# AlibabaResearch/recom

Measured on AMD Instinct MI355X. Metric: inference QPS + p50 latency, 1000-col synth model, batch 512, 1×MI355X, higher is better.
Workload: dtype f32; 1 GPU; S2: 1000 cols, dims 8/16/32/64, vocab 1000000, B 512, 1 id/row, 10% bucketize-f32, ids uniform; batch=512, columns=1000, table_bytes=120000000000, serve_workers=1, arena_ring=1

## Files before the change

### recom_amd/csrc/fcp_bench_main.hip

```cpp
#include <hip/hip_runtime.h>

#include <algorithm>
#include <atomic>
#include <thread>
#include <chrono>
#include <cmath>
#include <cstdint>
#include <cstdio>
#include <cstdlib>
#include <cstring>
#include <string>
#include <vector>

#include "../../include/fcp_hip.h"
#include "numa_util.h"

struct fcp_harness;
extern "C" int fcp_harness_create(fcp_plan_t *, const fcp_process_args_t *, int, int, int, fcp_harness **);
extern "C" int fcp_harness_run(fcp_harness *, int, double *, float *, float *);
extern "C" int fcp_harness_destroy(fcp_harness *);
extern "C" int fcp_harness_copy_probe(size_t, int, float *);
extern "C" int fcp_harness_bw_probe(int, size_t, int, float *);
extern "C" int fcp_harness_gather_probe(size_t, int, int, int, float *, double *);

#define CHECK_HIP(e)                                                                        \
  do {                                                                                      \
    hipError_t e_ = (e);                                                                    \
    if (e_ != hipSuccess) {                                                                 \
      std::fprintf(stderr, "%s:%d %s: %s\n", __FILE__, __LINE__, #e, hipGetErrorString(e_)); \
      std::exit(1);                                                                         \
    }                                                                                       \
  } while (0)
#define CHECK_FCP(e)                                                                                \
  do {                                                                                              \
    int s_ = (e);                                                                                   \
    if (s_) {                                                                                       \
      std::fprintf(stderr, "%s:%d %s: %s (%s)\n", __FILE__, __LINE__, #e, fcp_status_string(s_),   \
                   fcp_last_error());                                                               \
      std::exit(1);                                                                                 \
    }                                                                                               \
  } while (0)

__host__ __device__ inline float hash_elem(uint32_t seed, uint64_t r, uint32_t e) {
  uint64_t u = (r * 2654435761ull + (uint64_t)e * 40503ull + ((seed * 7919u + 12345u) & 0xFFFFFFFFull)) & 0xFFFFFFFFull;
  u ^= u >> 15;
  u = (u * 0x2C1B3C6Dull) & 0xFFFFFFFFull;
  u ^= u >> 12;
  u = (u * 0x297A2D39ull) & 0xFFFFFFFFull;
  u ^= u >> 15;
  return (float)(u >> 8) * 1.1920928955078125e-07f - 1.0f;
}

struct BigArg { char bytes[640]; };
__global__ void noop_big_kernel(BigArg a) { if (a.bytes[0] == 77) __builtin_trap(); }
__global__ void noop_kernel(int *p) { if (p) *p = 1; }

__global__ void fill_table(float *t, uint32_t seed, uint64_t vocab, uint32_t dim) {
  const uint64_t n = vocab * dim;
  for (uint64_t i = (uint64_t)blockIdx.x * blockDim.x + threadIdx.x; i < n; i += (uint64_t)gridDim.x * blockDim.x)
    t[i] = hash_elem(seed, i / dim, (uint32_t)(i % dim));
}

static uint64_t splitmix(uint64_t &s) {
  uint64_t z = (s += 0x9E3779B97F4A7C15ull);
  z = (z ^ (z >> 30)) * 0xBF58476D1CE4E5B9ull;
  z = (z ^ (z >> 27)) * 0x94D049BB133111EBull;
  return z ^ (z >> 31);
}

static int bucketize_host(const std::vector<float> &b, float v) {
  int l = 0, r = (int)b.size() - 1;
  while (l <= r) {
    int mid = (l + r) >> 1;
    if (v < b[mid]) r = mid - 1; else l = mid + 1;
  }
  return r + 1;
}

static void *plain_alloc(void *ctx, size_t bytes) {
  void **slot = static_cast<void **>(ctx);
  if (hipMalloc(slot, bytes) != hipSuccess) return nullptr;
  return *slot;
}

int main(int argc, char **argv) {
  int columns = 1000, batch = 512, steps = 300, warmup = 50, threads = 1, requests = 16, ring = 6, verify = 1;
  int bucketize_every = 10;
  int slab = 0;
  int h2d = 0;
  int narrow = 0;
  int zero_copy = std::getenv("FCP_STAGER_ZERO_COPY") ? 1 : 0;
  int fixed_dim = 0;
  int pack_threads = 8;
  int stager_depth = 4;
  int copy_kernel = 1;
  long vocab = 1000000;
  for (int i = 1; i + 1 < argc; i += 2) {
    std::string k = argv[i];
    long v = std::atol(argv[i + 1]);
    if (k == "--columns") columns = (int)v;
    else if (k == "--batch") batch = (int)v;
    else if (k == "--vocab") vocab = v;
    else if (k == "--steps") steps = (int)v;
    else if (k == "--warmup") warmup = (int)v;
    else if (k == "--threads") threads = (int)v;
    else if (k == "--requests") requests = (int)v;
    else if (k == "--ring") ring = (int)v;
    else if (k == "--verify") verify = (int)v;
    else if (k == "--bucketize-every") bucketize_every = (int)v;
    else if (k == "--slab") slab = (int)v;
    else if (k == "--h2d") h2d = (int)v;
    else if (k == "--narrow") narrow = (int)v;
    else if (k == "--zero-copy") zero_copy = (int)v;
    else if (k == "--dim") fixed_dim = (int)v;
    else if (k == "--pack-threads") pack_threads = (int)v;
    else if (k == "--stager-depth") stager_depth = (int)v;
    else if (k == "--copy-kernel") copy_kernel = (int)v;
    else if (k == "--bw-probe") {
      const char *names[4] = {"read", "write", "write-nt", "chunked-write-nt"};
      for (int kind = 0; kind < 4; ++kind) {
        float ms = 0;
        const size_t bytes = (size_t)v << 20;
        fcp_harness_bw_probe(kind, bytes, 20, &ms);
        std::printf("%s probe %ld MiB: %.1f GB/s  (%.2f us)\n", names[kind], v, bytes / (ms * 1e-3) / 1e9, ms * 1e3);
      }
      return 0;
    }
    else if (k == "--gather-probe") {
      for (int row_bytes : {32, 64, 128, 256}) {
        for (int depth : {4, 8}) {
          float ms = 0;
          double useful = 0;
          fcp_harness_gather_probe((size_t)v << 20, row_bytes, depth, 10, &ms, &useful);
          std::printf("gather probe %ld MiB, %3d-byte rows, %d in flight: %.1f GB/s useful (%.2f us per launch)\n", v, row_bytes,
                      depth, useful / (ms * 1e-3) / 1e9, ms * 1e3);
        }
      }
      return 0;
    }
    else if (k == "--api-probe") {
      hipStream_t s1, s2;
      hipEvent_t e1, e2;
      CHECK_HIP(hipStreamCreateWithFlags(&s1, hipStreamNonBlocking));
      CHECK_HIP(hipStreamCreateWithFlags(&s2, hipStreamNonBlocking));
      CHECK_HIP(hipEventCreateWithFlags(&e1, hipEventDisableTiming));
      CHECK_HIP(hipEventCreateWithFlags(&e2, hipEventDisableTiming));
      const int n = (int)v;
      auto now = [] { return std::chrono::steady_clock::now(); };
      auto us = [&](std::chrono::steady_clock::time_point a) { return std::chrono::duration<double, std::micro>(now() - a).count() / n; };
      {
        hipFunction_t f = nullptr;
        CHECK_HIP(hipGetFuncBySymbol(&f, reinterpret_cast<const void *>(noop_big_kernel)));
        BigArg arg;
        std::memset(&arg, 0, sizeof(arg));
        size_t arg_size = sizeof(arg);
        void *extra[] = {HIP_LAUNCH_PARAM_BUFFER_POINTER, &arg, HIP_LAUNCH_PARAM_BUFFER_SIZE, &arg_size, HIP_LAUNCH_PARAM_END};
        auto t = now();
        for (int i = 0; i < n; ++i) hipLaunchKernelGGL(noop_big_kernel, dim3(1), dim3(64), 0, s1, arg);
        std::printf("hipLaunchKernelGGL, 640-byte argument    %.2f us\n", us(t));
        CHECK_HIP(hipStreamSynchronize(s1));
        t = now();
        for (int i = 0; i < n; ++i) CHECK_HIP(hipModuleLaunchKernel(f, 1, 1, 1, 64, 1, 1, 0, s1, nullptr, extra));
        std::printf("hipModuleLaunchKernel, same argument     %.2f us\n", us(t));
        CHECK_HIP(hipStreamSynchronize(s1));
      }
      auto t = now();
      for (int i = 0; i < n; ++i) hipLaunchKernelGGL(noop_kernel, dim3(1), dim3(64), 0, s1, nullptr);
      std::printf("kernel launch          %.2f us\n", us(t));
      CHECK_HIP(hipDeviceSynchronize());
      t = now();
// ... 117 lines not shown
        } else {
          int64_t id = (int64_t)(splitmix(rng) % (uint64_t)vocab);
          std::memcpy(p + 8 * b, &id, 8);
        }
      }
    }
    CHECK_HIP(hipMalloc(&d_blobs[v], size));
    CHECK_HIP(hipMemcpy(d_blobs[v], blobs[v].data(), size, hipMemcpyHostToDevice));
    fcp_process_args_t &a = variants[v];
    std::memset(&a, 0, sizeof(a));
    a.concated_inputs = d_blobs[v];
    a.concated_bytes = (int64_t)size;
    a.concated_offsets = offs[v].data();
    a.concated_shapes = shps[v].data();
    a.input_ptrs = tables.data();
  }

  if (verify) {
    void *arena = nullptr;
    fcp_process_args_t a = variants[0];
    a.malloc_buff = plain_alloc;
    a.malloc_buff_ctx = &arena;
    std::vector<void *> gp(1);
    std::vector<int32_t> gs(2);
    fcp_process_result_t res;
    std::memset(&res, 0, sizeof(res));
    res.group_ptrs = gp.data();
    res.group_shapes = gs.data();
    CHECK_FCP(fcp_process_feature_columns(plan, &a, &res));
    CHECK_HIP(hipDeviceSynchronize());
    const size_t W = gs[1];
    std::vector<float> out((size_t)batch * W);
    CHECK_HIP(hipMemcpy(out.data(), gp[0], out.size() * 4, hipMemcpyDeviceToHost));
    size_t bad = 0, off = 0;
    for (int c = 0; c < columns; ++c) {
      const char *p = blobs[0].data() + offs[0][c];
      for (int b = 0; b < batch; ++b) {
        int64_t id;
        if (esz[c] == 4) {
          float x;
          std::memcpy(&x, p + 4 * b, 4);
          id = bucketize_host(boundaries, x);
        } else {
          std::memcpy(&id, p + 8 * b, 8);
        }
        for (int e = 0; e < cols[c].dim; ++e)
          if (out[(size_t)b * W + off + e] != hash_elem(1000 + c, (uint64_t)id, e)) ++bad;
      }
      off += cols[c].dim;
    }
    std::printf("verify: %zu mismatching elements of %zu\n", bad, out.size());
    CHECK_HIP(hipFree(arena));
    if (bad) return 3;
  }

  if (h2d) {
    {
      cpu_set_t near;
      if (!std::getenv("FCP_STAGER_NO_PIN") && fcp::cpus_near_device(0, &near)) (void)sched_setaffinity(0, sizeof(near), &near);
    }
    std::vector<uint8_t> nflags(columns, 0);
    size_t shipped = blobs[0].size();
    if (narrow) {
      shipped = 0;
      for (int c = 0; c < columns; ++c) {
        if (cols[c].id_source == FCP_IDS_I64) {
          cols[c].id_source = FCP_IDS_I32;
          esz[c] = 4;
          nflags[c] = 1;
        }
        shipped += (size_t)batch * 4;
      }
      CHECK_FCP(fcp_plan_destroy(plan));
      CHECK_FCP(fcp_plan_create(&pd, &plan));
      for (int c = 0; c < columns; ++c)
        if (nflags[c]) esz[c] = 8;
    }
    std::vector<std::vector<fcp_host_tensor_t>> host(requests, std::vector<fcp_host_tensor_t>(columns));
    std::vector<int64_t> dims(1, batch);
    for (int v = 0; v < requests; ++v)
      for (int c = 0; c < columns; ++c) host[v][c] = {blobs[v].data() + offs[v][c], esz[c], 1, dims.data()};
    int64_t arena_bytes = 0;
    CHECK_FCP(fcp_plan_arena_bytes(plan, shps[0].data(), nullptr, &arena_bytes));
    struct RingCtx { std::vector<void *> *r; size_t i; };
    struct Worker {
      fcp_stager_t *st = nullptr;
      hipStream_t stream = nullptr;
      std::vector<void *> ring;
      RingCtx rc{nullptr, 0};
      double host_stage_us = 0, host_process_us = 0;
    };
    const int nw = threads < 1 ? 1 : threads;
    std::vector<Worker> W(nw);
    for (Worker &w : W) {
      CHECK_FCP(fcp_stager_create_ex(0, (int64_t)blobs[0].size() + 4096, columns, columns, stager_depth, pack_threads,
                                     zero_copy ? FCP_STAGER_ZERO_COPY : copy_kernel ? FCP_STAGER_COPY_KERNEL : FCP_STAGER_COPY_SDMA, &w.st));
      w.ring.resize(6);
      for (auto &p : w.ring) CHECK_HIP(hipMalloc(&p, (size_t)arena_bytes));
      w.rc.r = &w.ring;
      CHECK_HIP(hipStreamCreateWithFlags(&w.stream, hipStreamNonBlocking));
    }
    auto one = [&](Worker &w, int k) {
      const int v = k % requests;
      fcp_process_args_t a;
      std::memset(&a, 0, sizeof(a));
      const auto h0 = std::chrono::steady_clock::now();
// ... 105 lines not shown
```

### recom_amd/csrc/fcp_dense_plain.hip

```cpp
#include "fcp_fused_bodies.h"

namespace {

template <int R> struct PlainLds {
  static constexpr int RB = FCP_WAVES_PER_BLOCK * R;
  static constexpr int IDS = RB + 1;
  static constexpr int REC = sizeof(FcpPlainSpan) + FCP_WAVE * sizeof(FcpPlainCol);
  alignas(16) char rec[REC];
  uint32_t off[FCP_WAVE * IDS];
};
static_assert(sizeof(FcpPlainCol) == 48 && sizeof(FcpPlainSpan) == 80, "span records: 80-byte head, 48-byte columns");

typedef uint32_t __attribute__((ext_vector_type(2))) U2;
typedef U2 __attribute__((aligned(4))) Id64;

template <int R>
__global__ void __launch_bounds__(FCP_BLOCK_THREADS)
fcp_dense_kernel_plain(const char *img, const char *blob, float *out, unsigned long long *bad_ids, int rows, int nslots,
                       int nsp8, int nlist, int img_stride, int out_stride, int policy) {
  constexpr int V = 4, RB = PlainLds<R>::RB, IDS = PlainLds<R>::IDS;
  __shared__ PlainLds<R> S;
  const int tid = threadIdx.x;
  const int lane = tid & (FCP_WAVE - 1);
  const int wave = tid >> 6;

  const int bid = blockIdx.x;
  int idx, tile;
  if (nsp8 > 0) {
    const int xcd = bid & 7, j8 = bid >> 3;
    idx = (j8 % nsp8) * 8 + xcd;
    tile = j8 / nsp8;
  } else {
    idx = bid % (-nsp8);
    tile = bid / (-nsp8);
  }
  if (idx >= nlist) return;
  const int q0 = idx * FCP_WAVE, row_blk = tile * RB;
  if (q0 >= nslots || row_blk >= rows) return;

  typedef uint32_t __attribute__((ext_vector_type(4))) U4;
  {
    const FCP_GLOBAL U4 *g = as_global(reinterpret_cast<const U4 *>(img + (int64_t)idx * img_stride));
    if (tid < (img_stride >> 4)) reinterpret_cast<U4 *>(S.rec)[tid] = g[tid];
  }
  __syncthreads();
  const FcpPlainSpan &H = *reinterpret_cast<const FcpPlainSpan *>(S.rec);
  const FcpPlainCol *cols = reinterpret_cast<const FcpPlainCol *>(S.rec + sizeof(FcpPlainSpan));

  const int npairs = H.ncols * RB;
  for (int p = tid; p < npairs; p += FCP_BLOCK_THREADS) {
    const int j = p / RB, r = p % RB;
    const int b = row_blk + r;
    uint32_t off = kNoRow;
    if (b < rows) {
      const FcpPlainCol &c = cols[j];
      const char *a = blob + c.ids_off;
      const uint32_t kind = c.kind;
      int64_t id;
      if (kind == FCP_IDS_I64) {
        const Id64 w = ((const FCP_GLOBAL Id64 *)a)[b];
        id = (int64_t)(((uint64_t)w.y << 32) | w.x);
      } else {
        const uint32_t w = *as_global(reinterpret_cast<const uint32_t *>(a) + b);
        id = kind == FCP_IDS_F32_BUCKETIZE ? (int64_t)bucketize_arith(c.n_boundaries, c.bnd_b0, c.bnd_inv, c.bnd_step, __uint_as_float(w))
                                           : (int64_t)(int32_t)w;
      }
      const bool bad = (uint64_t)id >= (uint64_t)c.vocab;
      off = bad ? kBadRow : (uint32_t)id * c.spr;
      if (bad && bad_ids && c.out_off >= q0 * V) atomicAdd(bad_ids, 1ull);
    }
    S.off[j * IDS + r] = off;
  }
  __syncthreads();
  const int q = q0 + lane;
  if (q >= nslots) return;

  const int j = H.lane_col[lane];
  const float *tb = cols[j].table + (q * V - cols[j].out_off);
  float *outp = out + q * V;
  const int r0 = wave * R;
  uint32_t off[R];
#pragma unroll
  for (int r = 0; r < R; ++r) off[r] = S.off[j * IDS + r0 + r];
  VF<V> v[R];
#pragma unroll
  for (int r = 0; r < R; ++r) {
    v[r] = vzero<V>();
    if (is_row(off[r])) v[r] = ld_slot32<V>(tb, off[r]);
  }
#pragma unroll
  for (int r = 0; r < R; ++r) {
    const int b = row_blk + r0 + r;
    if (b < rows) st_out<V>(outp + (int64_t)b * out_stride, v[r], policy);
  }
}

}

int fcp_launch_dense_plain(const FcpPlainLaunch &P, int grid_blocks, ihipStream_t *s) {
  if (grid_blocks <= 0) return 0;
  if (P.img_stride <= 0 || (P.img_stride & 15) || P.img_stride > PlainLds<4>::REC) return (int)hipErrorInvalidValue;
  void *stop = nullptr;
  int flags = 0;
  fcp_take_launch_extras(&stop, &flags);
  const dim3 grid(grid_blocks), block(FCP_BLOCK_THREADS);
  if (stop || flags)
    hipExtLaunchKernelGGL(fcp_dense_kernel_plain<4>, grid, block, 0, s, nullptr, static_cast<hipEvent_t>(stop), flags, P.img, P.blob,
                          P.out, P.bad_ids, P.rows, P.nslots, P.nsp8, P.nlist, P.img_stride, P.out_stride, P.store_policy);
  else
    hipLaunchKernelGGL(fcp_dense_kernel_plain<4>, grid, block, 0, s, P.img, P.blob, P.out, P.bad_ids, P.rows, P.nslots, P.nsp8,
                       P.nlist, P.img_stride, P.out_stride, P.store_policy);
  return (int)hipGetLastError();
}
```

### recom_amd/csrc/fcp_host.h

```cpp
#pragma once
#include <hip/hip_runtime.h>
#include <hip/hip_ext.h>

#include <algorithm>
#include <atomic>
#include <chrono>
#include <cmath>
#include <cstdio>
#include <cstdlib>
#include <cstring>
#include <functional>
#include <map>
#include <memory>
#include <mutex>
#include <new>
#include <string>
#include <thread>
#include <vector>

#include "../../include/fcp_hip.h"
#include "fcp_internal.h"
#include "fcp_env.h"

namespace fcph {
// ... 121 lines not shown
};
void sup_reset(LaneSupervisor &S, const fcp::Env &env);
LanePool *lane_pool_for(int device);

struct PendingResult {
  uintptr_t end;
  hipEvent_t done;
  const void *owner;
};
void pending_register(const void *owner, void *arena, int64_t bytes, const void *blob, int64_t blob_bytes, hipEvent_t done);
void pending_clear_range(void *arena, int64_t bytes);
void pending_forget(const void *owner);
int stager_input_wait(const void *base, int64_t bytes, hipStream_t stream);
int stager_input_synchronize(const void *base, int64_t bytes);
int wait_for_inputs(const void *const *inputs, int32_t n, void *stream);

}
using namespace fcph;

struct fcp_plan {
  fcp::Env env;
  fcp_plan_desc_t desc;
  std::vector<HostColumn> cols;
  std::vector<int32_t> ranks, elem_sizes, shape_off;
  std::vector<int32_t> group_width, group_nslots, group_map_off;
  std::vector<int32_t> seg_cols;
  int32_t n_seg_plain = 0;
  bool seg_search = false;
  bool has_inverse = false;
  bool csr_by_pos = false;
  std::vector<int32_t> order, pos_of;
  struct FastCol {
    int32_t ids_input, seg_input, rows_arg, dim, seg_stride;
    int64_t out_off_bytes;
    uint8_t form, rows_source, seg_kind, group;
  };
  std::vector<FastCol> fast_cols;
  std::vector<int32_t> group_rep;
  int vec = 1;
  bool dense_only = true;
  std::vector<uint32_t> span_list;
  std::vector<int32_t> list_off[2], list_n[2];
  uint32_t *d_span_list = nullptr;
  bool host_only = false;
  int32_t rank_sum = 0;

  uint32_t *d_slot_map = nullptr;
  FcpColStatic *d_cols = nullptr;
  FcpXform *d_xforms = nullptr;
  FcpSegMap *d_segmaps = nullptr;
  bool has_seg_map = false;
  bool has_weights = false, weighted_kernel = false;
  bool plain_dense = false;
  int32_t plain_stride = 0, plain_spans = 0;
  std::vector<char> plain_tmpl;
  std::vector<std::pair<uint32_t, int32_t>> plain_entries;
  std::atomic<int32_t> last_dense_front{0};
  bool wide_rows = false;
  int out_kind = FCP_OUT_F32, out_elem = 4;
  int tab_kind = FCP_TAB_F32, tab_elem = 4;
  int tab_row_tail = 0;
  std::vector<FcpColStatic> h_cols;
  char *d_const = nullptr;
  int32_t *d_seg_cols = nullptr;
  unsigned long long *d_bad = nullptr;
  float *d_zeros = nullptr;
  std::vector<const void *> bound_tables;
  bool tables_bound = false;

  bool host_writes_dyn = false;
  std::mutex mu;
  DynSlot slots[kSlots];
  uint64_t tick = 0;

  LanePool *pool = nullptr;
  uint32_t lane_flags = 0;
  std::vector<std::pair<void *, bool>> lane_verdicts;
  std::atomic<void *> lane_good_caller{nullptr};
  int32_t lane_count = 0;
  std::atomic<bool> lane_relies{false};
  std::atomic<int64_t> last_work_bytes{0};
  int64_t lane_min_work = 0;
  int32_t request_order = FCP_ORDER_STREAM;
  std::atomic<uintptr_t> recent_arena[2] = {};
  struct LastLaunch {
    std::atomic<int32_t> kernel{0}, rows_per_wave{0}, store_policy{0}, dense_blocks{0}, ragged_blocks{0}, segment_offsets{0};
    std::atomic<int64_t> csr_arena_off{-1};
    std::unique_ptr<std::atomic<int32_t>[]> csr_base;
  } last_launch;
  std::atomic<bool> lane_demoted{false};
  LaneSupervisor sup;
  std::atomic<bool> sup_window{false};
};

namespace fcph {

struct DeviceGuard {
  int prev = -1;
  bool changed = false;
  int enter(int dev) {
    hipError_t e = hipGetDevice(&prev);
    if (e != hipSuccess) return hip_fail("hipGetDevice", e);
    if (prev != dev) {
      e = hipSetDevice(dev);
      if (e != hipSuccess) return hip_fail("hipSetDevice", e);
      changed = true;
    }
// ... 45 lines not shown
```

### recom_amd/csrc/fcp_internal.h

```cpp
#pragma once
#include <stddef.h>
#include <stdint.h>

#ifndef FCP_MAX_GROUPS
#define FCP_MAX_GROUPS 16
#endif
#define FCP_BLOCK_THREADS 256
#define FCP_WAVES_PER_BLOCK 4
#define FCP_WAVE 64

#define FCP_F_FORM(f) ((f) & 0xFu)
#define FCP_F_COMBINER(f) (((f) >> 4) & 0xFu)
#define FCP_F_IDSRC(f) (((f) >> 8) & 0xFu)
#define FCP_F_SEGKIND(f) (((f) >> 12) & 0xFu)
#define FCP_F_PACK(form, comb, idsrc, segkind) \
  ((uint32_t)(form) | ((uint32_t)(comb) << 4) | ((uint32_t)(idsrc) << 8) | ((uint32_t)(segkind) << 12))

struct FcpColStatic {
  const float *table;
  const float *boundaries;
  int64_t vocab;
  int32_t dim;
  int32_t out_off;
  uint32_t flags;
// ... 23 lines not shown
  int32_t inner;
  int32_t rows;
  int32_t seg_sym;
};

struct FcpSegMap {
  int64_t mul[4];
  int64_t div;
  int32_t n;
  int32_t sym_slot;
};

struct FcpGroupLaunch {
  int32_t rows;
  int32_t nslots;
  int32_t nsp8;
  int32_t block_begin;
  int32_t slot_map_off;
  int32_t span_list_off;
  int32_t nlist;
  int32_t csr_reg_stride;
};

struct FcpLaunch {
  const uint32_t *slot_map;
  const uint32_t *span_list;
  const FcpColStatic *cols;
  const FcpColDyn *dyn;
  const char *blob;
  char *arena;
  unsigned long long *bad_ids;
  int64_t csr_arena_off;
  int32_t n_groups;
  int32_t rows_per_wave;
  int32_t shard_rank, shard_world;
  int32_t seg_search;
  int32_t store_through;
  const int32_t *csr_reg;
  FcpGroupLaunch groups[FCP_MAX_GROUPS];
  const FcpXform *xforms;
  const float *zeros;
};

struct FcpPlainCol {
  const float *table;
  int64_t ids_off;
  uint32_t vocab;
  uint32_t spr;
  int32_t out_off;
  uint32_t kind;
  int32_t n_boundaries;
  float bnd_b0, bnd_inv, bnd_step;
};
struct FcpPlainSpan {
  int32_t ncols;
  int32_t pad_[3];
  uint8_t lane_col[FCP_WAVE];
};
struct FcpPlainLaunch {
  const char *img;
  const char *blob;
  float *out;
  unsigned long long *bad_ids;
  int32_t rows, nslots, nsp8, nlist;
  int32_t img_stride;
  int32_t out_stride;
  int32_t store_policy;
};

struct FcpSegLaunch {
  const int32_t *seg_cols;
  const FcpColStatic *cols;
  const FcpColDyn *dyn;
  const char *blob;
  char *arena;
  int64_t csr_arena_off;
  unsigned long long *bad_ids;
  const FcpXform *xforms;
  const FcpSegMap *segmaps;
  int32_t skip_inverse;
};

struct ihipStream_t;
void fcp_set_stop_event(void *event);
bool fcp_stop_event_pending();
void fcp_set_any_order(bool on);
int fcp_launch_fused(const FcpLaunch &L, int vec, bool dense_kernel, int grid_blocks, ihipStream_t *s);
int fcp_launch_hybrid(const FcpLaunch &Ldense, int dense_blocks, const FcpLaunch &Lragged, int ragged_blocks, int vec,
                      ihipStream_t *s);
int fcp_launch_weighted(const FcpLaunch &L, const int64_t *wts, int vec, int grid_blocks, ihipStream_t *s);
int fcp_launch_narrow(const FcpLaunch &L, int vec, bool dense_kernel, int out_kind, int grid_blocks, ihipStream_t *s);
int fcp_launch_narrow_hybrid(const FcpLaunch &Ldense, int dense_blocks, const FcpLaunch &Lragged, int ragged_blocks, int vec,
                             int out_kind, ihipStream_t *s);
int fcp_launch_tab16(const FcpLaunch &L, int vec, bool dense_kernel, int tab_kind, int grid_blocks, ihipStream_t *s);
int fcp_launch_tab16_hybrid(const FcpLaunch &Ldense, int dense_blocks, const FcpLaunch &Lragged, int ragged_blocks, int vec,
                            int tab_kind, ihipStream_t *s);
int fcp_launch_tabq8(const FcpLaunch &L, int vec, bool dense_kernel, int grid_blocks, ihipStream_t *s);
int fcp_launch_tabq8_hybrid(const FcpLaunch &Ldense, int dense_blocks, const FcpLaunch &Lragged, int ragged_blocks, int vec,
                            ihipStream_t *s);
int fcp_launch_dense_plain(const FcpPlainLaunch &P, int grid_blocks, ihipStream_t *s);
void fcp_take_launch_extras(void **stop_event, int *flags);
int fcp_launch_upload(const void *host_mapped_src, void *dst, size_t bytes, ihipStream_t *s);
int fcp_launch_h2d_copy(const void *host_mapped_src, void *dst, size_t bytes, ihipStream_t *s);
int fcp_launch_segment_offsets(const FcpSegLaunch &L, int n_seg_cols, int max_nnz, ihipStream_t *s, bool any_order = false);
int fcp_launch_concat_outputs(const void *const *inputs, const int32_t *dims, const int32_t *col_offsets, const int32_t *in_strides,
                              int32_t n, int64_t prefix, int32_t width, int32_t first_off, void *out,
                              ihipStream_t *s);
int fcp_launch_shard_finalize(const FcpLaunch &L, int group, const float *partials, int world,
                              int64_t row_begin, int64_t row_count, float *out, int vec,
// ... 2 lines not shown
```

### recom_amd/csrc/fcp_plan.hip

```cpp
#include "fcp_host.h"

namespace fcph {

thread_local std::string g_last_error;

int hip_fail(const char *what, hipError_t e) {
  g_last_error = std::string(what) + ": " + hipGetErrorString(e);
  return (e == hipErrorNoDevice || e == hipErrorInvalidDevice || e == hipErrorNoBinaryForGpu ||
          e == hipErrorInsufficientDriver)
             ? FCP_ERR_NO_DEVICE
             : FCP_ERR_HIP;
}

int fail(int code, const std::string &msg) {
  g_last_error = msg;
  return code;
}

}

int fcp_internal_fail(int code, const std::string &msg) { return fail(code, msg); }

namespace fcph {

// ... 538 lines not shown
    return std::min(std::max(g, 0), n);
  };
  auto exact = [&](float x) { return (int)(std::upper_bound(b.begin(), b.end(), x) - b.begin()); };
  int misses = 0;
  for (int i = 0; i < n; ++i) {
    if (i && !(b[i] > b[i - 1])) return;
    const float below = std::nextafter(b[i], -INFINITY);
    misses += guess(b[i]) != exact(b[i]);
    misses += guess(below) != exact(below);
  }
  if (misses * 8 > n) return;
  *b0 = lo;
  *inv = scale;
  const float step = b[1] - b[0];
  if (!(step > 0.0f) || !std::isfinite(step)) return;
  for (int i = 0; i < n; ++i)
    if (std::fmaf((float)i, step, lo) != b[i]) return;
  *step_out = step;
}

void build_plain_template(fcp_plan *p) {
  p->plain_dense = false;
  if (fcp::diag_ll("dense_generic", 0) != 0) return;
  const fcp_plan_desc_t &d = p->desc;
  if (p->out_elem != 4 || p->tab_elem != 4 || d.layout != FCP_LAYOUT_CONCAT || d.n_groups != 1 || d.shard_world > 1 || p->vec != 4 || p->wide_rows ||
      p->weighted_kernel || !p->dense_only || p->cols.empty())
    return;
  const int nc = (int)p->cols.size();
  for (int pos = 0; pos < nc; ++pos) {
    const HostColumn &hc = p->cols[p->order[pos]];
    const FcpColStatic &s = p->h_cols[pos];
    if (hc.d.form != FCP_FORM_GATHER || s.xform != 0 || hc.d.vocab < 0 || hc.d.vocab >= 0xFFFFFFFDLL) return;
    if (hc.d.id_source == FCP_IDS_F32_BUCKETIZE) {
      if (s.bnd_step == 0.0f) return;
    } else if (hc.d.id_source != FCP_IDS_I32 && hc.d.id_source != FCP_IDS_I64) {
      return;
    }
  }
  const int nslots = p->group_nslots[0];
  const int nspans = (nslots + FCP_WAVE - 1) / FCP_WAVE;
  if (p->list_n[0][0] != nspans) return;
  std::vector<int> first(nspans, nc), last(nspans, -1);
  for (int pos = 0; pos < nc; ++pos) {
    const FcpColStatic &s = p->h_cols[pos];
    const int s0 = s.out_off / 4 / FCP_WAVE, s1 = (s.out_off + s.dim - 1) / 4 / FCP_WAVE;
    for (int sp = s0; sp <= s1; ++sp) {
      first[sp] = std::min(first[sp], pos);
      last[sp] = std::max(last[sp], pos);
    }
  }
  int max_cols = 1;
  for (int sp = 0; sp < nspans; ++sp) max_cols = std::max(max_cols, last[sp] - first[sp] + 1);
  if (max_cols > FCP_WAVE) return;
  p->plain_stride = (int32_t)(sizeof(FcpPlainSpan) + (size_t)max_cols * sizeof(FcpPlainCol));
  p->plain_spans = nspans;
  p->plain_tmpl.assign((size_t)nspans * p->plain_stride, 0);
  p->plain_entries.clear();
  for (int sp = 0; sp < nspans; ++sp) {
    char *rec = p->plain_tmpl.data() + (size_t)sp * p->plain_stride;
    FcpPlainSpan head;
    std::memset(&head, 0, sizeof(head));
    head.ncols = last[sp] - first[sp] + 1;
    for (int pos = first[sp]; pos <= last[sp]; ++pos) {
      const FcpColStatic &s = p->h_cols[pos];
      FcpPlainCol c;
      std::memset(&c, 0, sizeof(c));
      c.table = nullptr;
      c.ids_off = 0;
      c.vocab = (uint32_t)s.vocab;
      c.spr = (uint32_t)(s.dim / 4);
      c.out_off = s.out_off;
      c.kind = FCP_F_IDSRC(s.flags);
      c.n_boundaries = s.n_boundaries;
      c.bnd_b0 = s.bnd_b0;
      c.bnd_inv = s.bnd_inv;
      c.bnd_step = s.bnd_step;
      const size_t at = (size_t)sp * p->plain_stride + sizeof(FcpPlainSpan) + (size_t)(pos - first[sp]) * sizeof(FcpPlainCol);
      std::memcpy(p->plain_tmpl.data() + at, &c, sizeof(c));
      p->plain_entries.emplace_back((uint32_t)at, pos);
      for (int q = std::max(s.out_off / 4, sp * FCP_WAVE); q < std::min((s.out_off + s.dim) / 4, (sp + 1) * FCP_WAVE); ++q)
        head.lane_col[q - sp * FCP_WAVE] = (uint8_t)(pos - first[sp]);
    }
    std::memcpy(rec, &head, sizeof(head));
  }
  p->plain_dense = true;
}

void destroy_device(fcp_plan *p) {
  if (p->host_only) return;
  for (auto &s : p->slots) {
    if (s.h_dyn) (void)hipHostFree(s.h_dyn);
    if (s.d_dyn) (void)hipFree(s.d_dyn);
    if (s.uploaded) (void)hipEventDestroy(s.uploaded);
    for (auto &e : s.done_pool) (void)hipEventDestroy(e.second);
  }
  if (p->d_slot_map) (void)hipFree(p->d_slot_map);
  if (p->d_span_list) (void)hipFree(p->d_span_list);
  if (p->d_cols) (void)hipFree(p->d_cols);
  if (p->d_xforms) (void)hipFree(p->d_xforms);
  if (p->d_segmaps) (void)hipFree(p->d_segmaps);
  if (p->d_const) (void)hipFree(p->d_const);
  if (p->d_seg_cols) (void)hipFree(p->d_seg_cols);
  if (p->d_bad) (void)hipFree(p->d_bad);
  if (p->d_zeros) (void)hipFree(p->d_zeros);
}

int init_device(fcp_plan *p) {
  DeviceGuard guard;
  int rc = guard.enter(p->desc.device);
  if (rc) return rc;
  const int nc = (int)p->cols.size();
  std::vector<uint32_t> map;
  for (int g = 0; g < p->desc.n_groups; ++g) {
    p->group_map_off[g] = (int32_t)map.size();
    for (int pos = 0; pos < nc; ++pos) {
      const HostColumn &hc = p->cols[p->order[pos]];
      if (hc.d.concat_group != g) continue;
      for (int s = 0; s < hc.d.dim / p->vec; ++s) map.push_back((uint32_t)pos);
    }
  }
  HIP_TRY(hipMalloc(&p->d_span_list, std::max<size_t>(p->span_list.size(), 1) * sizeof(uint32_t)));
  HIP_TRY(hipMemcpy(p->d_span_list, p->span_list.data(), p->span_list.size() * sizeof(uint32_t), hipMemcpyHostToDevice));
  HIP_TRY(hipMalloc(&p->d_slot_map, std::max<size_t>(map.size(), 1) * sizeof(uint32_t)));
  HIP_TRY(hipMemcpy(p->d_slot_map, map.data(), map.size() * sizeof(uint32_t), hipMemcpyHostToDevice));
  int64_t const_bytes = 0;
  std::vector<int> owners;
  for (size_t k = 0; k < p->cols.size(); ++k) {
    HostColumn &hc = p->cols[k];
    if (hc.boundaries.empty()) continue;
    for (int o : owners)
// ... 806 lines not shown
```

### recom_amd/csrc/fcp_process.hip

```cpp
#include "fcp_host.h"

namespace fcph {

bool stream_is_capturing(hipStream_t stream) {
  hipStreamCaptureStatus st = hipStreamCaptureStatusNone;
  if (stream && hipStreamIsCapturing(stream, &st) == hipSuccess) return st == hipStreamCaptureStatusActive;
  (void)hipGetLastError();
  return false;
}

static void fill_plain_image(const fcp_plan *p, const FcpColStatic *cols, FcpColDyn *h_dyn) {
  char *img = reinterpret_cast<char *>(h_dyn) + slot_image_off(p);
  std::memcpy(img, p->plain_tmpl.data(), p->plain_tmpl.size());
  for (const auto &e : p->plain_entries) {
    FcpPlainCol *c = reinterpret_cast<FcpPlainCol *>(img + e.first);
    c->table = cols[e.second].table;
    c->ids_off = h_dyn[e.second].ids_off;
  }
}

int bind_tables(fcp_plan *p, const void *const *input_ptrs, bool capturing) {
  const int nt = p->desc.n_device_inputs;
  if (p->tables_bound && std::memcmp(p->bound_tables.data(), input_ptrs, nt * sizeof(void *)) == 0)
    return FCP_OK;
  if (capturing)
    return fail(FCP_ERR_UNSUPPORTED, "stream capture of a request whose tables are not bound to the plan yet (or have moved): run it "
                                     "once on this stream before capturing");
  std::vector<FcpColStatic> cols = p->h_cols;
  for (size_t k = 0; k < p->cols.size(); ++k) {
    const int t = p->cols[k].d.table_input;
    const bool lookup = p->cols[k].d.form == FCP_FORM_GATHER || p->cols[k].d.form == FCP_FORM_SEGMENT_REDUCE ||
                        p->cols[k].d.form == FCP_FORM_GATHER_SCATTER;
    if (lookup) {
      const bool empty_shard = p->desc.shard_world > 1 && p->cols[k].d.vocab <= p->desc.shard_rank;
      if (!input_ptrs[t] && !empty_shard) return fail(FCP_ERR_INVALID_ARGUMENT, "null table pointer");
      cols[p->pos_of[k]].table = static_cast<const float *>(input_ptrs[t]);
    }
  }
  if (p->tables_bound) HIP_TRY(hipDeviceSynchronize());
  p->tables_bound = false;
  HIP_TRY(hipMemcpy(p->d_cols, cols.data(), cols.size() * sizeof(FcpColStatic), hipMemcpyHostToDevice));
  p->h_cols.swap(cols);
  if (p->plain_dense) {
    for (auto &s : p->slots) {
      if (!s.img_built) continue;
      fill_plain_image(p, p->h_cols.data(), s.h_dyn);
      const size_t off = slot_image_off(p);
      HIP_TRY(hipMemcpy(reinterpret_cast<char *>(s.d_dyn) + off, reinterpret_cast<const char *>(s.h_dyn) + off, p->plain_tmpl.size(),
                        hipMemcpyHostToDevice));
    }
  }
  for (int t = 0; t < nt; ++t) p->bound_tables[t] = input_ptrs[t];
  p->tables_bound = true;
  return FCP_OK;
}

int done_event_for(DynSlot &s, void *stream) {
  s.done_gen = 0;
  for (auto &e : s.done_pool)
    if (e.first == stream) {
      s.done = e.second;
      return FCP_OK;
    }
  hipEvent_t ev = nullptr;
  HIP_TRY(hipEventCreateWithFlags(&ev, hipEventDisableTiming | hipEventDisableSystemFence));
  s.done_pool.emplace_back(stream, ev);
  s.done = ev;
  return FCP_OK;
}

void build_key(const fcp_plan *p, const fcp_process_args_t *a, std::vector<int32_t> &key) {
  const int nh = (int)p->ranks.size();
  const int nsym = a->symbols ? p->desc.n_symbols : 0;
  const size_t key_len = (size_t)nh + p->rank_sum + nsym + 3;
  key.resize(key_len);
  std::memcpy(key.data(), a->concated_offsets, nh * sizeof(int32_t));
  std::memcpy(key.data() + nh, a->concated_shapes, p->rank_sum * sizeof(int32_t));
  if (nsym) std::memcpy(key.data() + nh + p->rank_sum, a->symbols, nsym * sizeof(int32_t));
  key[key_len - 3] = (int32_t)std::min<int64_t>(a->concated_bytes, 0x7fffffff);
  const uint64_t stream_bits = (uint64_t)reinterpret_cast<uintptr_t>(a->stream);
  key[key_len - 2] = (int32_t)(uint32_t)stream_bits;
  key[key_len - 1] = (int32_t)(uint32_t)(stream_bits >> 32);
}

int find_or_reserve(fcp_plan *p, const std::vector<int32_t> &key, DynSlot **out, bool *install, bool capturing) {
  ++p->tick;
  DynSlot *victim = nullptr;
  int pinned = 0;
  for (auto &s : p->slots) {
    if (s.valid && s.key == key) {
      s.tick = p->tick;
      ++s.users;
      ++s.uses;
      s.done_valid = false;
      if (capturing) s.captured = true;
      *out = &s;
      *install = false;
      return FCP_OK;
    }
    if (s.captured) {
      ++pinned;
      continue;
    }
    if (s.users > 0) continue;
    auto rank = [](const DynSlot &x) { return !x.valid ? 0 : (x.done_valid ? 1 : 2); };
    if (!victim || rank(s) < rank(*victim) || (rank(s) == rank(*victim) && s.tick < victim->tick)) victim = &s;
  }
  if (capturing) return kNeedsInstall;
  if (!victim)
    return pinned == kSlots ? fail(FCP_ERR_UNSUPPORTED, "every descriptor slot belongs to a captured graph: fcp_plan_release_captures")
                            : kAllSlotsBusy;
  victim->was_valid = victim->valid;
  victim->img_built = false;
  victim->valid = false;
  victim->users = 1;
  *out = victim;
  *install = true;
  return FCP_OK;
}

int install_slot(fcp_plan *p, const fcp_process_args_t *a, DynSlot &s) {
  hipStream_t stream = static_cast<hipStream_t>(a->stream);
  if (s.was_valid) {
    if (!s.done_valid) {
      if (s.stream == a->stream) {
        HIP_TRY(hipStreamSynchronize(stream));
      } else {
        HIP_TRY(hipDeviceSynchronize());
      }
    } else if (s.done_gen != 0 && s.done_gen != g_lane_generation.load(std::memory_order_acquire)) {
    } else if (hipEventQuery(s.done) != hipSuccess) {
      HIP_TRY(hipEventSynchronize(s.done));
    }
    if (!p->host_writes_dyn && hipEventQuery(s.uploaded) != hipSuccess) HIP_TRY(hipEventSynchronize(s.uploaded));
  }
  int rc = compute_dyn(p, a->concated_offsets, a->concated_shapes, a->symbols, a->concated_bytes, s.h_dyn, &s.meta);
  if (rc) return rc;
  if (p->has_weights) {
    rc = compute_weights(p, a->concated_offsets, a->concated_shapes, reinterpret_cast<int64_t *>(s.h_dyn + p->cols.size()));
    if (rc) return rc;
  }
  p->last_work_bytes.store(s.meta.work_bytes, std::memory_order_relaxed);
  s.meta.plain = p->plain_dense && s.meta.geo[0].rows_per_wave == 4 && s.meta.geo[1].grid_blocks == 0 &&
                 s.meta.geo[0].groups[0].span_list_off < 0 && s.meta.geo[0].groups[0].nlist == p->plain_spans;
  std::unique_lock<std::mutex> image_lock(p->mu, std::defer_lock);
  if (s.meta.plain) {
    image_lock.lock();
    fill_plain_image(p, p->h_cols.data(), s.h_dyn);
    s.img_built = true;
  }
  const size_t dyn_bytes = s.meta.plain ? slot_dyn_bytes(p) : (slot_dyn_bytes(p) - (p->plain_dense ? p->plain_tmpl.size() : 0));
  if (p->host_writes_dyn) {
    std::memcpy(s.d_dyn, s.h_dyn, dyn_bytes);
    __builtin_ia32_sfence();
  } else {
    const int e = fcp_launch_upload(s.h_dyn_dev, s.d_dyn, dyn_bytes, stream);
    if (e) return hip_fail("descriptor upload launch", (hipError_t)e);
    HIP_TRY(hipEventRecord(s.uploaded, stream));
  }
  return done_event_for(s, a->stream);
}

void publish_slot(fcp_plan *p, DynSlot &s, const std::vector<int32_t> &key, void *stream) {
  s.done_valid = false;
  s.uses = 1;
  s.key = key;
  s.stream = stream;
  s.tick = p->tick;
  s.valid = true;
}

int store_policy_for(fcp_plan *p, const void *arena, int64_t out_bytes) {
  const int64_t through_bytes = p->env.store_through_bytes;
  const uintptr_t ar = reinterpret_cast<uintptr_t>(arena);
  const uintptr_t a0 = p->recent_arena[0].load(std::memory_order_relaxed), a1 = p->recent_arena[1].load(std::memory_order_relaxed);
  const bool reused = ar == a0 || ar == a1;
  if (ar != a0) {
    p->recent_arena[1].store(a0, std::memory_order_relaxed);
    p->recent_arena[0].store(ar, std::memory_order_relaxed);
  }
  constexpr int64_t kPlainMaxBytes = (int64_t)160 << 20;
  if (out_bytes < through_bytes) return 0;
  return (reused && out_bytes <= kPlainMaxBytes) ? 4 : 1;
}

void fill_launch(const fcp_plan *p, const DynSlot &s, int kind, const void *blob, void *arena, int store_policy, FcpLaunch *L) {
  L->slot_map = p->d_slot_map;
  L->span_list = p->d_span_list;
  L->cols = p->d_cols;
  L->xforms = p->d_xforms;
  L->zeros = p->d_zeros;
  L->dyn = s.d_dyn;
  L->blob = static_cast<const char *>(blob);
  L->arena = static_cast<char *>(arena);
  L->bad_ids = p->d_bad;
  L->csr_arena_off = s.meta.csr_arena_off;
  L->shard_rank = p->desc.shard_rank;
  L->shard_world = p->desc.shard_world;
  L->n_groups = p->desc.n_groups;
  L->rows_per_wave = s.meta.geo[kind].rows_per_wave;
  L->seg_search = s.meta.seg_search ? 1 : 0;
  L->store_through = store_policy | (p->wide_rows ? 2 : 0);
// ... 253 lines not shown
```

Baseline: 19.14 million inferences/s.

## Pack per-column id facts into span records and prefetch ids before LDS sync

Each plain-dense span record gains a packed array of 32-bit id facts, holding the id offset and id kind per column. Each thread reads these through the constant path and issues its first id load before the record is staged to LDS and before the barrier. Later passes of the pair loop then stride over columns without per-pair divisions or dependent loads from the LDS column record. This aims to hide id-load latency and trim the descriptor chain at kernel start. In exchange the record grows by the facts area, and the host falls back to the non-plain path when an id offset is unaligned or too large. A separate mix-probe benchmark kernel is added for measuring store policies.

Measured after the change: 19.71 million inferences/s (median of 6 runs). 1.03x the previous value.

```diff
diff --git a/recom_amd/csrc/fcp_bench_main.hip b/recom_amd/csrc/fcp_bench_main.hip
--- a/recom_amd/csrc/fcp_bench_main.hip
+++ b/recom_amd/csrc/fcp_bench_main.hip
@@ -13,6 +13,7 @@
 #include <vector>
 
 #include "../../include/fcp_hip.h"
+#include "fcp_fused_bodies.h"
 #include "numa_util.h"
 
 struct fcp_harness;
@@ -61,6 +62,41 @@
     t[i] = hash_elem(seed, i / dim, (uint32_t)(i % dim));
 }
 
+__global__ void __launch_bounds__(FCP_BLOCK_THREADS)
+mix_probe_kernel(const float *const *tptr, const uint32_t *roff, const int32_t *col_of, int roff_stride, float *out, int rows, int nslots,
+                 int nsp8, int nlist, int out_stride, int policy) {
+  constexpr int V = 4, R = 4, RB = FCP_WAVES_PER_BLOCK * R;
+  const int lane = threadIdx.x & (FCP_WAVE - 1), wave = threadIdx.x >> 6;
+  const int bid = blockIdx.x;
+  int idx, tile;
+  if (nsp8 > 0) {
+    const int xcd = bid & 7, j8 = bid >> 3;
+    idx = (j8 % nsp8) * 8 + xcd;
+    tile = j8 / nsp8;
+  } else {
+    idx = bid % (-nsp8);
+    tile = bid / (-nsp8);
+  }
+  if (idx >= nlist) return;
+  const int q = idx * FCP_WAVE + lane, row0 = tile * RB + wave * R;
+  if (q >= nslots || row0 >= rows) return;
+  const float *tb = *as_global(tptr + q);
+  uint32_t off[R];
+  const int at = col_of ? *as_global(col_of + q) : q;
+#pragma unroll
+  for (int r = 0; r < R; ++r) off[r] = row0 + r < rows ? *as_global(roff + (int64_t)(row0 + r) * roff_stride + at) : kNoRow;
+  VF<V> v[R];
+#pragma unroll
+  for (int r = 0; r < R; ++r) {
+    v[r] = vzero<V>();
+    if (is_row(off[r])) v[r] = ld_slot32<V>(tb, off[r]);
+  }
+  float *outp = out + q * V;
+#pragma unroll
+  for (int r = 0; r < R; ++r)
+    if (row0 + r < rows) st_out<V>(outp + (int64_t)(row0 + r) * out_stride, v[r], policy);
+}
+
 static uint64_t splitmix(uint64_t &s) {
   uint64_t z = (s += 0x9E3779B97F4A7C15ull);
   z = (z ^ (z >> 30)) * 0xBF58476D1CE4E5B9ull;
@@ -94,6 +130,7 @@
   int pack_threads = 8;
   int stager_depth = 4;
   int copy_kernel = 1;
+  int mix_probe = 0;
   long vocab = 1000000;
   for (int i = 1; i + 1 < argc; i += 2) {
     std::string k = argv[i];
@@ -116,6 +153,7 @@
     else if (k == "--pack-threads") pack_threads = (int)v;
     else if (k == "--stager-depth") stager_depth = (int)v;
     else if (k == "--copy-kernel") copy_kernel = (int)v;
+    else if (k == "--mix-probe") mix_probe = (int)v;
     else if (k == "--bw-probe") {
       const char *names[4] = {"read", "write", "write-nt", "chunked-write-nt"};
       for (int kind = 0; kind < 4; ++kind) {
@@ -339,6 +377,115 @@
     std::printf("verify: %zu mismatching elements of %zu\n", bad, out.size());
     CHECK_HIP(hipFree(arena));
     if (bad) return 3;
+  }
+
+  if (mix_probe) {
+    int width = 0;
+    std::vector<int> out_off(columns);
+    for (int c = 0; c < columns; ++c) {
+      out_off[c] = width;
+      width += cols[c].dim;
+    }
+    const int nslots = width / 4, nspans = (nslots + FCP_WAVE - 1) / FCP_WAVE;
+    const int nsp8 = nspans >= 8 ? (nspans + 7) / 8 : -nspans, ntiles = (batch + 15) / 16;
+    const int grid = (nsp8 > 0 ? 8 * nsp8 : nspans) * ntiles;
+    std::vector<const float *> h_tptr(nslots);
+    std::vector<int> col_of(nslots);
+    for (int c = 0; c < columns; ++c)
+      for (int q = out_off[c] / 4; q < (out_off[c] + cols[c].dim) / 4; ++q) {
+        col_of[q] = c;
+        h_tptr[q] = static_cast<const float *>(tables[c]) + (q * 4 - out_off[c]);
+      }
+    const float **d_tptr = nullptr;
+    CHECK_HIP(hipMalloc(reinterpret_cast<void **>(&d_tptr), nslots * sizeof(float *)));
+    CHECK_HIP(hipMemcpy(d_tptr, h_tptr.data(), nslots * sizeof(float *), hipMemcpyHostToDevice));
+    std::vector<uint32_t *> d_roff(requests);
+    const bool compact = mix_probe == 2;
+    const int roff_stride = compact ? columns : nslots;
+    int32_t *d_col_of = nullptr;
+    if (compact) {
+      CHECK_HIP(hipMalloc(reinterpret_cast<void **>(&d_col_of), nslots * sizeof(int32_t)));
+      CHECK_HIP(hipMemcpy(d_col_of, col_of.data(), nslots * sizeof(int32_t), hipMemcpyHostToDevice));
+    }
+    std::vector<uint32_t> h_roff((size_t)batch * roff_stride), col_row(columns);
+    for (int v = 0; v < requests; ++v) {
+      for (int b = 0; b < batch; ++b) {
+        for (int c = 0; c < columns; ++c) {
+          const char *p = blobs[v].data() + offs[v][c];
+          int64_t id;
+          if (esz[c] == 4) {
+            float x;
+            std::memcpy(&x, p + 4 * b, 4);
+            id = bucketize_host(boundaries, x);
+          } else {
+            std::memcpy(&id, p + 8 * b, 8);
+          }
+          col_row[c] = (uint32_t)id * (uint32_t)(cols[c].dim / 4);
+        }
+        for (int k = 0; k < roff_stride; ++k) h_roff[(size_t)b * roff_stride + k] = col_row[compact ? k : col_of[k]];
+      }
+      CHECK_HIP(hipMalloc(reinterpret_cast<void **>(&d_roff[v]), h_roff.size() * 4));
+      CHECK_HIP(hipMemcpy(d_roff[v], h_roff.data(), h_roff.size() * 4, hipMemcpyHostToDevice));
+    }
+    const size_t out_bytes = (size_t)batch * width * 4;
+    std::vector<float *> arenas(6);
+    for (auto &a : arenas) CHECK_HIP(hipMalloc(reinterpret_cast<void **>(&a), out_bytes));
+    hipStream_t st;
+    hipEvent_t e0, e1;
+    CHECK_HIP(hipStreamCreateWithFlags(&st, hipStreamNonBlocking));
+    CHECK_HIP(hipEventCreate(&e0));
+    CHECK_HIP(hipEventCreate(&e1));
+    if (verify) {
+      hipLaunchKernelGGL(mix_probe_kernel, dim3(grid), dim3(FCP_BLOCK_THREADS), 0, st, d_tptr, d_roff[0], d_col_of, roff_stride, arenas[0], batch,
+                         nslots, nsp8, nspans, width, 0);
+      CHECK_HIP(hipStreamSynchronize(st));
+      std::vector<float> out((size_t)batch * width);
+      CHECK_HIP(hipMemcpy(out.data(), arenas[0], out_bytes, hipMemcpyDeviceToHost));
+      size_t bad = 0;
+      for (int b = 0; b < batch; ++b)
+        for (int q = 0; q < nslots; ++q) {
+          const int c = col_of[q];
+          const char *p = blobs[0].data() + offs[0][c];
+          int64_t id;
+          if (esz[c] == 4) {
+            float x;
+            std::memcpy(&x, p + 4 * b, 4);
+            id = bucketize_host(boundaries, x);
+          } else {
+            std::memcpy(&id, p + 8 * b, 8);
+          }
+          for (int e = 0; e < 4; ++e)
+            if (out[(size_t)b * width + q * 4 + e] != hash_elem(1000 + c, (uint64_t)id, q * 4 - out_off[c] + e)) ++bad;
+        }
+      std::printf("mix probe verify: %zu mismatching elements of %zu\n", bad, out.size());
+      if (bad) return 3;
+    }
+    double line_bytes = 0;
+    for (int c = 0; c < columns; ++c) line_bytes += (double)batch * ((cols[c].dim * 4 + 127) / 128 * 128);
+    std::printf("mix probe %d: grid %d x %d, %d slots, %d rows; per launch %.1f MB of table lines + %.1f MB of output + %.1f MB of offsets\n",
+                mix_probe, grid, FCP_BLOCK_THREADS, nslots, batch, line_bytes / 1e6, (double)batch * width * 4 / 1e6,
+                (double)batch * roff_stride * 4 / 1e6);
+    const char *names[3] = {"nt", "sc1 nt", "plain"};
+    const int policies[3] = {0, FCP_ST_THROUGH, FCP_ST_PLAIN};
+    for (int pass = 0; pass < 2; ++pass)
+      for (int nring : {1, 6})
+        for (int k = 0; k < 3; ++k) {
+          auto run = [&](int n) {
+            for (int i = 0; i < n; ++i)
+              hipLaunchKernelGGL(mix_probe_kernel, dim3(grid), dim3(FCP_BLOCK_THREADS), 0, st, d_tptr, d_roff[i % requests],
+                                 d_col_of, roff_stride, arenas[i % nring], batch, nslots, nsp8, nspans, width, policies[k]);
+          };
+          run(warmup > 0 ? warmup : 1);
+          CHECK_HIP(hipEventRecord(e0, st));
+          run(steps);
+          CHECK_HIP(hipEventRecord(e1, st));
+          CHECK_HIP(hipEventSynchronize(e1));
+          CHECK_HIP(hipGetLastError());
+          float ms = 0;
+          CHECK_HIP(hipEventElapsedTime(&ms, e0, e1));
+          std::printf("mix probe %d pass %d ring %d stores %-6s  %.3f us per launch\n", mix_probe, pass, nring, names[k], ms * 1e3 / steps);
+        }
+    return 0;
   }
 
   if (h2d) {
diff --git a/recom_amd/csrc/fcp_dense_plain.hip b/recom_amd/csrc/fcp_dense_plain.hip
--- a/recom_amd/csrc/fcp_dense_plain.hip
+++ b/recom_amd/csrc/fcp_dense_plain.hip
@@ -5,11 +5,16 @@
 template <int R> struct PlainLds {
   static constexpr int RB = FCP_WAVES_PER_BLOCK * R;
   static constexpr int IDS = RB + 1;
-  static constexpr int REC = sizeof(FcpPlainSpan) + FCP_WAVE * sizeof(FcpPlainCol);
+  static constexpr int REC = FCP_PLAIN_FACTS_OFF + fcp_plain_facts_bytes(FCP_WAVE) + FCP_WAVE * sizeof(FcpPlainCol);
   alignas(16) char rec[REC];
   uint32_t off[FCP_WAVE * IDS];
 };
-static_assert(sizeof(FcpPlainCol) == 48 && sizeof(FcpPlainSpan) == 80, "span records: 80-byte head, 48-byte columns");
+static_assert(sizeof(FcpPlainCol) == 48 && sizeof(FcpPlainSpan) == FCP_PLAIN_FACTS_OFF && FCP_PLAIN_FACTS_OFF % 16 == 0 &&
+                  fcp_plain_facts_bytes(1) == 64 && fcp_plain_facts_bytes(FCP_WAVE) == 256,
+              "span records: 80-byte head, id facts in whole passes of 16 dwords, 48-byte columns");
+static_assert(FCP_BLOCK_THREADS / (FCP_WAVES_PER_BLOCK * 4) == FCP_PLAIN_FACTS_PER_PASS && FCP_WAVE / (FCP_WAVES_PER_BLOCK * 4) == 4,
+              "R = 4: a pass of the pair loop covers 16 columns, a wave four");
+static_assert(PlainLds<4>::REC / 16 <= FCP_BLOCK_THREADS, "one 16-byte piece of the record per thread");
 
 typedef uint32_t __attribute__((ext_vector_type(2))) U2;
 typedef U2 __attribute__((aligned(4))) Id64;
@@ -39,37 +44,56 @@
   if (q0 >= nslots || row_blk >= rows) return;
 
   typedef uint32_t __attribute__((ext_vector_type(4))) U4;
-  {
-    const FCP_GLOBAL U4 *g = as_global(reinterpret_cast<const U4 *>(img + (int64_t)idx * img_stride));
-    if (tid < (img_stride >> 4)) reinterpret_cast<U4 *>(S.rec)[tid] = g[tid];
-  }
+  const char *rec = img + (int64_t)idx * img_stride;
+  const FCP_CONST U4 *facts = (const FCP_CONST U4 *)(rec + FCP_PLAIN_FACTS_OFF) + __builtin_amdgcn_readfirstlane(wave);
+  const U4 f0 = *facts;
+  const bool rec_thread = tid < (img_stride >> 4);
+  U4 rec_regs = {0, 0, 0, 0};
+  if (rec_thread) rec_regs = as_global(reinterpret_cast<const U4 *>(rec))[tid];
+
+  const int r = tid % RB, b = row_blk + r;
+  const int sub = lane / RB;
+  const int bc = b < rows ? b : rows - 1;
+  auto load_id = [&](U4 f, uint32_t &kind) -> U2 {
+    const uint32_t lo2 = (sub & 1) ? f.y : f.x, hi2 = (sub & 1) ? f.w : f.z;
+    const uint32_t fact = (sub & 2) ? hi2 : lo2;
+    kind = b < rows ? fact >> 30 : FCP_PLAIN_FACT_NONE;
+    const bool wide = (fact >> 30) == FCP_PLAIN_FACT_I64;
+    const FCP_GLOBAL uint32_t *a = as_global(reinterpret_cast<const uint32_t *>(blob + ((uint64_t)(fact & 0x3FFFFFFFu) << 2))) + (wide ? 2 * bc : bc);
+    U2 w;
+    w.x = a[0];
+    w.y = a[wide ? 1 : 0];
+    return w;
+  };
+  uint32_t kind;
+  U2 w = load_id(f0, kind);
+  if (rec_thread) reinterpret_cast<U4 *>(S.rec)[tid] = rec_regs;
   __syncthreads();
   const FcpPlainSpan &H = *reinterpret_cast<const FcpPlainSpan *>(S.rec);
-  const FcpPlainCol *cols = reinterpret_cast<const FcpPlainCol *>(S.rec + sizeof(FcpPlainSpan));
+  const FcpPlainCol *cols = reinterpret_cast<const FcpPlainCol *>(S.rec + H.cols_off);
 
-  const int npairs = H.ncols * RB;
-  for (int p = tid; p < npairs; p += FCP_BLOCK_THREADS) {
-    const int j = p / RB, r = p % RB;
-    const int b = row_blk + r;
-    uint32_t off = kNoRow;
-    if (b < rows) {
-      const FcpPlainCol &c = cols[j];
-      const char *a = blob + c.ids_off;
-      const uint32_t kind = c.kind;
-      int64_t id;
-      if (kind == FCP_IDS_I64) {
-        const Id64 w = ((const FCP_GLOBAL Id64 *)a)[b];
-        id = (int64_t)(((uint64_t)w.y << 32) | w.x);
-      } else {
-        const uint32_t w = *as_global(reinterpret_cast<const uint32_t *>(a) + b);
-        id = kind == FCP_IDS_F32_BUCKETIZE ? (int64_t)bucketize_arith(c.n_boundaries, c.bnd_b0, c.bnd_inv, c.bnd_step, __uint_as_float(w))
-                                           : (int64_t)(int32_t)w;
+  const int ncols = H.ncols;
+  for (int j = tid / RB;;) {
+    if (j < ncols) {
+      uint32_t off = kNoRow;
+      if (kind != FCP_PLAIN_FACT_NONE) {
+        const FcpPlainCol &c = cols[j];
+        int64_t id;
+        if (kind == FCP_PLAIN_FACT_I64)
+          id = (int64_t)(((uint64_t)w.y << 32) | w.x);
+        else
+          id = kind == FCP_PLAIN_FACT_F32 ? (int64_t)bucketize_arith(c.n_boundaries, c.bnd_b0, c.bnd_inv, c.bnd_step, __uint_as_float(w.x))
+                                          : (int64_t)(int32_t)w.x;
+        const bool bad = (uint64_t)id >= (uint64_t)c.vocab;
+        off = bad ? kBadRow : (uint32_t)id * c.spr;
+        if (bad && bad_ids && c.out_off >= q0 * V) atomicAdd(bad_ids, 1ull);
       }
-      const bool bad = (uint64_t)id >= (uint64_t)c.vocab;
-      off = bad ? kBadRow : (uint32_t)id * c.spr;
-      if (bad && bad_ids && c.out_off >= q0 * V) atomicAdd(bad_ids, 1ull);
+      S.off[j * IDS + r] = off;
     }
-    S.off[j * IDS + r] = off;
+    j += FCP_PLAIN_FACTS_PER_PASS;
+    if (j - sub >= ncols) break;
+    facts += FCP_BLOCK_THREADS / FCP_WAVE;
+    w = load_id(*facts, kind);
   }
   __syncthreads();
   const int q = q0 + lane;
@@ -99,7 +123,9 @@
 
 int fcp_launch_dense_plain(const FcpPlainLaunch &P, int grid_blocks, ihipStream_t *s) {
   if (grid_blocks <= 0) return 0;
-  if (P.img_stride <= 0 || (P.img_stride & 15) || P.img_stride > PlainLds<4>::REC) return (int)hipErrorInvalidValue;
+  if (P.img_stride < FCP_PLAIN_FACTS_OFF + fcp_plain_facts_bytes(1) + (int)sizeof(FcpPlainCol) || (P.img_stride & 15) ||
+      P.img_stride > PlainLds<4>::REC)
+    return (int)hipErrorInvalidValue;
   void *stop = nullptr;
   int flags = 0;
   fcp_take_launch_extras(&stop, &flags);
diff --git a/recom_amd/csrc/fcp_host.h b/recom_amd/csrc/fcp_host.h
--- a/recom_amd/csrc/fcp_host.h
+++ b/recom_amd/csrc/fcp_host.h
@@ -197,7 +197,7 @@
   bool has_seg_map = false;
   bool has_weights = false, weighted_kernel = false;
   bool plain_dense = false;
-  int32_t plain_stride = 0, plain_spans = 0;
+  int32_t plain_stride = 0, plain_spans = 0, plain_cols_off = 0;
   std::vector<char> plain_tmpl;
   std::vector<std::pair<uint32_t, int32_t>> plain_entries;
   std::atomic<int32_t> last_dense_front{0};
diff --git a/recom_amd/csrc/fcp_internal.h b/recom_amd/csrc/fcp_internal.h
--- a/recom_amd/csrc/fcp_internal.h
+++ b/recom_amd/csrc/fcp_internal.h
@@ -99,9 +99,16 @@
   int32_t n_boundaries;
   float bnd_b0, bnd_inv, bnd_step;
 };
+constexpr uint32_t FCP_PLAIN_FACT_NONE = 0, FCP_PLAIN_FACT_I32 = 1, FCP_PLAIN_FACT_I64 = 2, FCP_PLAIN_FACT_F32 = 3;
+constexpr int FCP_PLAIN_FACTS_OFF = 80;
+constexpr int FCP_PLAIN_FACTS_PER_PASS = 16;
+constexpr int fcp_plain_facts_bytes(int max_cols) {
+  return (max_cols + FCP_PLAIN_FACTS_PER_PASS - 1) / FCP_PLAIN_FACTS_PER_PASS * FCP_PLAIN_FACTS_PER_PASS * 4;
+}
 struct FcpPlainSpan {
   int32_t ncols;
-  int32_t pad_[3];
+  int32_t cols_off;
+  int32_t pad_[2];
   uint8_t lane_col[FCP_WAVE];
 };
 struct FcpPlainLaunch {
diff --git a/recom_amd/csrc/fcp_plan.hip b/recom_amd/csrc/fcp_plan.hip
--- a/recom_amd/csrc/fcp_plan.hip
+++ b/recom_amd/csrc/fcp_plan.hip
@@ -614,7 +614,8 @@
   int max_cols = 1;
   for (int sp = 0; sp < nspans; ++sp) max_cols = std::max(max_cols, last[sp] - first[sp] + 1);
   if (max_cols > FCP_WAVE) return;
-  p->plain_stride = (int32_t)(sizeof(FcpPlainSpan) + (size_t)max_cols * sizeof(FcpPlainCol));
+  p->plain_cols_off = FCP_PLAIN_FACTS_OFF + fcp_plain_facts_bytes(max_cols);
+  p->plain_stride = (int32_t)(p->plain_cols_off + (size_t)max_cols * sizeof(FcpPlainCol));
   p->plain_spans = nspans;
   p->plain_tmpl.assign((size_t)nspans * p->plain_stride, 0);
   p->plain_entries.clear();
@@ -623,6 +624,7 @@
     FcpPlainSpan head;
     std::memset(&head, 0, sizeof(head));
     head.ncols = last[sp] - first[sp] + 1;
+    head.cols_off = p->plain_cols_off;
     for (int pos = first[sp]; pos <= last[sp]; ++pos) {
       const FcpColStatic &s = p->h_cols[pos];
       FcpPlainCol c;
@@ -637,7 +639,7 @@
       c.bnd_b0 = s.bnd_b0;
       c.bnd_inv = s.bnd_inv;
       c.bnd_step = s.bnd_step;
-      const size_t at = (size_t)sp * p->plain_stride + sizeof(FcpPlainSpan) + (size_t)(pos - first[sp]) * sizeof(FcpPlainCol);
+      const size_t at = (size_t)sp * p->plain_stride + p->plain_cols_off + (size_t)(pos - first[sp]) * sizeof(FcpPlainCol);
       std::memcpy(p->plain_tmpl.data() + at, &c, sizeof(c));
       p->plain_entries.emplace_back((uint32_t)at, pos);
       for (int q = std::max(s.out_off / 4, sp * FCP_WAVE); q < std::min((s.out_off + s.dim) / 4, (sp + 1) * FCP_WAVE); ++q)
diff --git a/recom_amd/csrc/fcp_process.hip b/recom_amd/csrc/fcp_process.hip
--- a/recom_amd/csrc/fcp_process.hip
+++ b/recom_amd/csrc/fcp_process.hip
@@ -9,14 +9,21 @@
   return false;
 }
 
-static void fill_plain_image(const fcp_plan *p, const FcpColStatic *cols, FcpColDyn *h_dyn) {
+static bool fill_plain_image(const fcp_plan *p, const FcpColStatic *cols, FcpColDyn *h_dyn) {
   char *img = reinterpret_cast<char *>(h_dyn) + slot_image_off(p);
   std::memcpy(img, p->plain_tmpl.data(), p->plain_tmpl.size());
   for (const auto &e : p->plain_entries) {
     FcpPlainCol *c = reinterpret_cast<FcpPlainCol *>(img + e.first);
     c->table = cols[e.second].table;
     c->ids_off = h_dyn[e.second].ids_off;
-  }
+    const uint64_t off = (uint64_t)c->ids_off;
+    if ((off & 3) || (off >> 32)) return false;
+    const uint32_t rec = e.first / (uint32_t)p->plain_stride * (uint32_t)p->plain_stride;
+    const uint32_t j = (e.first - rec - (uint32_t)p->plain_cols_off) / (uint32_t)sizeof(FcpPlainCol);
+    const uint32_t kind = c->kind == FCP_IDS_I64 ? FCP_PLAIN_FACT_I64 : c->kind == FCP_IDS_I32 ? FCP_PLAIN_FACT_I32 : FCP_PLAIN_FACT_F32;
+    reinterpret_cast<uint32_t *>(img + rec + FCP_PLAIN_FACTS_OFF)[j] = (uint32_t)(off >> 2) | kind << 30;
+  }
+  return true;
 }
 
 int bind_tables(fcp_plan *p, const void *const *input_ptrs, bool capturing) {
@@ -44,7 +51,7 @@
   if (p->plain_dense) {
     for (auto &s : p->slots) {
       if (!s.img_built) continue;
-      fill_plain_image(p, p->h_cols.data(), s.h_dyn);
+      (void)fill_plain_image(p, p->h_cols.data(), s.h_dyn);
       const size_t off = slot_image_off(p);
       HIP_TRY(hipMemcpy(reinterpret_cast<char *>(s.d_dyn) + off, reinterpret_cast<const char *>(s.h_dyn) + off, p->plain_tmpl.size(),
                         hipMemcpyHostToDevice));
@@ -146,8 +153,9 @@
   std::unique_lock<std::mutex> image_lock(p->mu, std::defer_lock);
   if (s.meta.plain) {
     image_lock.lock();
-    fill_plain_image(p, p->h_cols.data(), s.h_dyn);
-    s.img_built = true;
+    s.meta.plain = fill_plain_image(p, p->h_cols.data(), s.h_dyn);
+    s.img_built = s.meta.plain;
+    if (!s.meta.plain) image_lock.unlock();
   }
   const size_t dyn_bytes = s.meta.plain ? slot_dyn_bytes(p) : (slot_dyn_bytes(p) - (p->plain_dense ? p->plain_tmpl.size() : 0));
   if (p->host_writes_dyn) {
```
